# TinfoilHat0/Defending-Against-Backdoors-with-Robust-Learning-Rate

Measured on AMD Instinct MI355X. Metric: fl_rounds_per_sec, higher is better.
Workload: dtype fp32; 1 GPU; model=CNN_MNIST, dataset=fmnist (synthetic, 6000 samples/agent), num_agents=10, agents_per_gpu=10, num_corrupt=1, robustLR_threshold=4, aggr=avg, local_ep=2, global_batch=256, parallelism=dp1 (agent-sharded, RCCL all-gather)

## Files before the change

rlr_amd/ops/csrc/bindings.cpp:

```cpp
#include <torch/extension.h>
#include <c10/hip/HIPStream.h>

#include <algorithm>
#include <cstdint>
#include <vector>

#include "launchers.h"

#define CHK(x) TORCH_CHECK(x, #x)
#define CHK_CUDA(t)                                                      \
  TORCH_CHECK((t).is_cuda() &&                                           \
                  ((t).is_contiguous() ||                                \
                   (t).is_contiguous(torch::MemoryFormat::ChannelsLast)),\
              #t " must be cuda + dense")

static void* stream_of(const torch::Tensor& t) {
  return (void*)c10::hip::getCurrentHIPStream(t.device().index()).stream();
}

static bool layout_debug() {
  static int v = -1;
  if (v < 0) {
    const char* e = getenv("RLR_AMD_DEBUG_LAYOUT");
    v = (e && e[0] == '1') ? 1 : 0;
// ... 1326 lines not shown
                                  torch::Tensor dw_out,
                                  c10::optional<torch::Tensor> relu_y) {
  TORCH_CHECK(x.is_cuda());
  TORCH_CHECK(dw_out.is_contiguous() && dw_out.numel() == w.numel());
  return conv_bwd_core(x, w, dy, stride, pad, need_dx, dw_out, c10::nullopt,
                       relu_y);
}


std::tuple<torch::Tensor, torch::Tensor, torch::Tensor> batchnorm_fwd(
    torch::Tensor x, torch::Tensor w, torch::Tensor b,
    torch::Tensor running_mean, torch::Tensor running_var, double momentum,
    double eps, bool training, bool relu) {
  TORCH_CHECK(x.is_cuda());
  x = cl(x, "bn_fwd.x");
  int Nb = x.size(0), C = x.size(1), HW = x.size(2) * x.size(3);
  auto y = empty_cl({x.size(0), x.size(1), x.size(2), x.size(3)},
                    x.options());
  auto save_mean = torch::empty({C}, x.options().dtype(torch::kFloat));
  auto save_rstd = torch::empty({C}, x.options().dtype(torch::kFloat));
  auto scratch = torch::empty({(long)bn_scratch_floats(C)},
                              x.options().dtype(torch::kFloat));
  if (is_bf16(x))
    launch_bn_fwd_bf16(bfc(x), w.data_ptr<float>(), b.data_ptr<float>(),
                       running_mean.data_ptr<float>(),
                       running_var.data_ptr<float>(),
                       save_mean.data_ptr<float>(),
                       save_rstd.data_ptr<float>(), bfp(y),
                       scratch.data_ptr<float>(), Nb, C, HW,
                       (float)momentum, (float)eps, training ? 1 : 0,
                       relu ? 1 : 0, stream_of(x));
  else
    launch_bn_fwd(x.data_ptr<float>(), w.data_ptr<float>(),
                  b.data_ptr<float>(), running_mean.data_ptr<float>(),
                  running_var.data_ptr<float>(),
                  save_mean.data_ptr<float>(), save_rstd.data_ptr<float>(),
                  y.data_ptr<float>(), scratch.data_ptr<float>(), Nb, C,
                  HW, (float)momentum, (float)eps, training ? 1 : 0,
                  relu ? 1 : 0, stream_of(x));
  return {y, save_mean, save_rstd};
}

torch::Tensor batchnorm_bwd_into(torch::Tensor x, torch::Tensor w,
                                 torch::Tensor save_mean,
                                 torch::Tensor save_rstd, torch::Tensor dy,
                                 torch::Tensor dw_out, torch::Tensor db_out) {
  TORCH_CHECK(x.is_cuda());
  x = cl(x, "bn_bwd.x");
  dy = cl(dy, "bn_bwd.dy");
  int Nb = x.size(0), C = x.size(1), HW = x.size(2) * x.size(3);
  TORCH_CHECK(dw_out.is_contiguous() && dw_out.numel() == C);
  TORCH_CHECK(db_out.is_contiguous() && db_out.numel() == C);
  auto dx = empty_cl({x.size(0), x.size(1), x.size(2), x.size(3)},
                     x.options());
  auto scratch = torch::empty({(long)bn_scratch_floats(C)},
                              x.options().dtype(torch::kFloat));
  if (is_bf16(x))
    launch_bn_bwd_bf16(bfc(x), bfc(dy), w.data_ptr<float>(),
                       save_mean.data_ptr<float>(),
                       save_rstd.data_ptr<float>(),
                       scratch.data_ptr<float>(), bfp(dx),
                       dw_out.data_ptr<float>(), db_out.data_ptr<float>(),
                       Nb, C, HW, 1, stream_of(x));
  else
    launch_bn_bwd(x.data_ptr<float>(), dy.data_ptr<float>(),
                  w.data_ptr<float>(), save_mean.data_ptr<float>(),
                  save_rstd.data_ptr<float>(), scratch.data_ptr<float>(),
                  dx.data_ptr<float>(), dw_out.data_ptr<float>(),
                  db_out.data_ptr<float>(), Nb, C, HW, 1, stream_of(x));
  return dx;
}

std::tuple<torch::Tensor, torch::Tensor, torch::Tensor> batchnorm_bwd(
    torch::Tensor x, torch::Tensor w, torch::Tensor save_mean,
    torch::Tensor save_rstd, torch::Tensor dy) {
  auto f32 = x.options().dtype(torch::kFloat);
  auto dw = torch::empty({x.size(1)}, f32);
  auto db = torch::empty({x.size(1)}, f32);
  auto dx = batchnorm_bwd_into(x, w, save_mean, save_rstd, dy, dw, db);
  return {dx, dw, db};
}


void poison_set_u8(torch::Tensor data, torch::Tensor idxs,
                   torch::Tensor coords, int64_t value) {
  CHK_CUDA(data);
  int H = data.size(1), W = data.size(2);
  int C = data.dim() == 4 ? data.size(3) : 1;
  launch_poison_set_u8(data.data_ptr<uint8_t>(), idxs.data_ptr<int64_t>(),
                       idxs.numel(), coords.data_ptr<int>(),
                       coords.size(0), H, W, C, (int)value, stream_of(data));
}

void poison_set_f32(torch::Tensor data, torch::Tensor idxs,
                    torch::Tensor coords, double value) {
  CHK_CUDA(data);
  int H = data.size(2), W = data.size(3);
  launch_poison_set_f32(data.data_ptr<float>(), idxs.data_ptr<int64_t>(),
                        idxs.numel(), coords.data_ptr<int>(),
                        coords.size(0), H, W, (float)value, stream_of(data));
}

void poison_addwrap_u8(torch::Tensor data, torch::Tensor idxs,
                       torch::Tensor mask) {
  CHK_CUDA(data);
  launch_poison_addwrap_u8(data.data_ptr<uint8_t>(),
                           idxs.data_ptr<int64_t>(), idxs.numel(),
                           mask.data_ptr<uint8_t>(),
                           data.size(1) * data.size(2), stream_of(data));
}

void poison_subf(torch::Tensor data, torch::Tensor idxs,
                 torch::Tensor mask) {
  CHK_CUDA(data);
  long HW = data.numel() / data.size(0);
  launch_poison_subf(data.data_ptr<float>(), idxs.data_ptr<int64_t>(),
                     idxs.numel(), mask.data_ptr<uint8_t>(), (int)HW,
                     stream_of(data));
}

torch::Tensor normalize_u8(torch::Tensor raw, torch::Tensor mean,
                           torch::Tensor stdv) {
  TORCH_CHECK(raw.is_cuda() && raw.is_contiguous());
  long B = raw.size(0);
  int H = raw.size(1), W = raw.size(2);
  int C = raw.dim() == 4 ? raw.size(3) : 1;
  auto out = empty_cl({B, C, H, W}, raw.options().dtype(torch::kFloat32));
  launch_normalize_u8(raw.data_ptr<uint8_t>(), out.data_ptr<float>(), B, H,
                      W, C, mean.data_ptr<float>(), stdv.data_ptr<float>(),
                      stream_of(raw));
  return out;
}


std::vector<torch::Tensor> prep_conv_weights(
    std::vector<std::pair<torch::Tensor, int64_t>> items) {
  StepQueue q;
  std::vector<torch::Tensor> out;
  out.reserve(items.size());
  for (auto& it : items) out.push_back(q.wperm(it.first, it.second));
  q.flush();
  return out;
}

void feed_gather(torch::Tensor X, torch::Tensor Y, torch::Tensor sel,
                 torch::Tensor out_x, torch::Tensor out_y) {
  StepQueue q;
  q.gather_rows(X, sel, out_x);
  q.gather_rows(Y, sel, out_y);
  q.flush();
}

torch::Tensor conv_db(torch::Tensor dy) {
  TORCH_CHECK(dy.is_cuda() && dy.dim() == 4 && !is_bf16(dy));
  dy = cl(dy, "conv_db.dy");
  auto db = torch::empty({dy.size(1)}, dy.options());
  StepQueue(true).conv_db(dy, db);
  return db;
}

torch::Tensor splitk_reduce_dwperm(torch::Tensor ws, int64_t Kout, int64_t C,
                                   int64_t RS, int64_t SK) {
  CHK_CUDA(ws);
  TORCH_CHECK(ws.numel() >= conv_dwperm_ws_floats(Kout, C * RS, SK));
  auto dw = torch::empty({Kout * C * RS}, ws.options());
  StepQueue(true).splitk_reduce_dwperm(ws, dw, Kout, C, RS, SK, 0);
  return dw;
}

torch::Tensor splitk_reduce(torch::Tensor ws, int64_t M, int64_t N,
                            int64_t SK) {
  CHK_CUDA(ws);
  TORCH_CHECK(ws.numel() >= gemm_splitk_ws_floats(M, N, SK));
  auto C = torch::empty({M, N}, ws.options());
  if (!StepQueue(true).splitk_reduce(ws, C, c10::nullopt, M, N, N, SK, false))
    launch_splitk_reduce(ws.data_ptr<float>(), C.data_ptr<float>(), nullptr,
                         (int)M, (int)N, (int)N, (int)SK, 0, stream_of(ws));
  return C;
}

torch::Tensor conv_small_bwdw_reduce(torch::Tensor partials, int64_t Nb,
                                     int64_t C, int64_t Kout, int64_t R,
                                     int64_t S, int64_t OH, int64_t OW) {
  CHK_CUDA(partials);
  auto dw = torch::empty({Kout * C * R * S}, partials.options());
  StepQueue(true).conv_small_bwdw_reduce(partials, dw, Nb, C, Kout, R, S, OH,
                                         OW);
  return dw;
}

torch::Tensor colsum(torch::Tensor dy) {
  CHK_CUDA(dy);
  TORCH_CHECK(dy.dim() == 2);
  auto db = torch::empty({dy.size(1)}, dy.options());
  StepQueue(true).colsum(dy, db);
  return db;
}

torch::Tensor wperm(torch::Tensor w, int64_t kind) {
  TORCH_CHECK(w.is_cuda());
  return StepQueue(true).wperm(w, kind);
}

std::tuple<std::vector<int64_t>, int64_t> step_batch_plan_py(
    std::vector<int64_t> counts) {
  std::vector<int> c(counts.begin(), counts.end()), f(counts.size());
  int total = step_batch_plan(c.data(), (int)c.size(), f.data());
  return {std::vector<int64_t>(f.begin(), f.end()), (int64_t)total};
}

std::tuple<int64_t, int64_t> step_batch_lookup_py(std::vector<int64_t> counts,
                                                  int64_t block) {
  std::vector<int> c(counts.begin(), counts.end());
  int v = -1;
  int r = step_batch_lookup(c.data(), (int)c.size(), (int)block, &v);
  return {(int64_t)r, (int64_t)(r < 0 ? -1 : v)};
}

}

PYBIND11_MODULE(TORCH_EXTENSION_NAME, m) {
  m.def("relu_fwd", &relu_fwd);
  m.def("relu_bwd", &relu_bwd);
  m.def("add_relu_fwd", &add_relu_fwd);
  m.def("maxpool2x2_fwd", &maxpool2x2_fwd);
  m.def("maxpool2x2_bwd", &maxpool2x2_bwd);
  m.def("dropout_fwd", &dropout_fwd);
  m.def("dropout_fwd_dev", &dropout_fwd_dev);
  m.def("dropout_bwd", &dropout_bwd);
  m.def("gap_fwd", &gap_fwd);
  m.def("gap_bwd", &gap_bwd);
  m.def("cross_entropy_fwd", &cross_entropy_fwd);
  m.def("cross_entropy_bwd", &cross_entropy_bwd);
  m.def("eval_update", &eval_update);
  m.def("clipped_sgd_step", &clipped_sgd_step);
  m.def("pgd_project", &pgd_project);
  m.def("delta64", &delta64);
  m.def("gather_grads", &gather_grads);
  m.def("fused_avg_rlr_apply", &fused_avg_rlr_apply, py::arg("U"),
        py::arg("w"), py::arg("params"), py::arg("rlr"), py::arg("thresh"),
        py::arg("slr"), py::arg("noise_std"), py::arg("seed"),
        py::arg("offset"), py::arg("want_lr"), py::arg("divisor") = 0.0);
  m.def("rlr_vote", &rlr_vote);
  m.def("agg_avg", &agg_avg, py::arg("U"), py::arg("w"),
        py::arg("divisor") = 0.0);
  m.def("agg_sign", &agg_sign);
  m.def("agg_comed", &agg_comed);
  m.def("apply_update", &apply_update);
  m.def("agg_orderstat", &agg_orderstat);
  m.def("orderstat_rlr_apply", &orderstat_rlr_apply);
  m.def("orderstat_max_k", &orderstat_max_k);
  m.def("bulyan_trim", &bulyan_trim);
  m.def("bulyan_rlr_apply", &bulyan_rlr_apply);
  m.def("bulyan_max_k", &bulyan_max_k);
  m.def("pairwise_sqdist", &pairwise_sqdist);
  m.def("pairdist_max_k", &pairdist_max_k);
  m.def("pairdist_chunks", &pairdist_chunks);
  m.def("pairdist_ws_doubles", &pairdist_ws_doubles);
  m.def("rows_add_", &rows_add_);
  m.def("gram_rows", &gram_rows);
  m.def("foolsgold_weights", &foolsgold_weights);
  m.def("foolsgold_max_k", &foolsgold_max_k);
  m.def("geomed_sqdist", &geomed_sqdist);
  m.def("geomed_weights", &geomed_weights);
  m.def("geomed_max_k", &geomed_max_k);
  m.def("geomed_chunks", &geomed_chunks);
  m.def("geomed_ws_doubles", &geomed_ws_doubles);
  m.def("rownorm_partials", &rownorm_partials);
  m.def("row_norms", &row_norms, py::arg("U"), py::arg("ws") = py::none());
  m.def("rowclip_", &rowclip_, py::arg("U"), py::arg("value"),
        py::arg("median_mode"), py::arg("ws") = py::none());
  m.def("rownorm_chunks", &rownorm_chunks);
  m.def("rownorm_ws_doubles", &rownorm_ws_doubles);
  m.def("gemm", &gemm);
  m.def("gemm_bf16", &gemm_bf16);
  m.def("nhwc_flatten", &nhwc_flatten);
  m.def("nhwc_unflatten", &nhwc_unflatten);
  m.def("linear_fwd", &linear_fwd);
  m.def("linear_bwd", &linear_bwd);
  m.def("conv2d_fwd", &conv2d_fwd, py::arg("x"), py::arg("w"), py::arg("b"),
        py::arg("stride"), py::arg("pad"), py::arg("relu"),
        py::arg("wt") = py::none());
  m.def("conv2d_pool_fwd", &conv2d_pool_fwd, py::arg("x"), py::arg("w"),
        py::arg("b"), py::arg("stride"), py::arg("pad"),
        py::arg("wt") = py::none());
  m.def("conv_pool_fused_ok", &conv_pool_fused_ok);
  m.def("conv_fwd_res_plan", [](int C, int H, int W, int OH, int OW, int R) {
    ConvFwdResPlan p = conv_fwd_res_plan(C, H, W, OH, OW, R);
    return std::make_tuple(p.tile_rows, p.tiles, p.mi, p.lds_rows,
                           p.lds_bytes);
  });
  m.def("conv2d_bwd", &conv2d_bwd);
  m.def("conv2d_bwd_into", &conv2d_bwd_into, py::arg("x"), py::arg("w"),
        py::arg("dy"), py::arg("stride"), py::arg("pad"), py::arg("need_dx"),
        py::arg("dw_out"), py::arg("db_out"), py::arg("relu_y"),
        py::arg("wp") = py::none(), py::arg("queue") = py::none());
  m.def("linear_bwd_into", &linear_bwd_into, py::arg("x"), py::arg("w"),
        py::arg("dy"), py::arg("dw_out"), py::arg("db_out"),
        py::arg("need_dx"), py::arg("queue") = py::none());
  m.def("dropout_relu_bwd", &dropout_relu_bwd);
  m.def("batchnorm_bwd_into", &batchnorm_bwd_into);
  m.def("conv2d_bwd_wdx_into", &conv2d_bwd_wdx_into);
  m.def("gemm_f32_splitk", &gemm_f32_splitk);
  m.def("conv_bwd_weight_splitk", &conv_bwd_weight_splitk);
  m.def("conv_bwd_weight_bf16_splitk", &conv_bwd_weight_bf16_splitk);
  m.def("conv_db_chunks", &conv_db_chunks);
  m.def("gemm_splitk_ws_floats", &gemm_splitk_ws_floats);
  m.def("conv_bwd_weight_ws_floats", &conv_bwd_weight_ws_floats);
  m.def("conv_dwperm_ws_floats", &conv_dwperm_ws_floats);
  m.def("conv_db_ws_floats", &conv_db_ws_floats);
  m.def("flat_norm_scratch_floats", &flat_norm_scratch_floats);
  m.def("conv_bwdw_tap_ws_slabs", [](int64_t Nb, int64_t C, int64_t Kout) {
    int S, G, chunks;
    int slabs = conv_bwdw_tap_ws_slabs((int)Nb, (int)C, (int)Kout, &S, &G,
                                       &chunks);
    return std::make_tuple(S, G, chunks, slabs);
  });
  m.def("conv_tap_fwd_ok", [](int a, int b, int c, int d, int e, int f,
                              int g, int h) {
    return conv_tap_fwd_ok(a, b, c, d, e, f, g, h) != 0;
  });
  m.def("conv_tap_fwd_w4_ok", [](int a, int b, int c, int d, int e, int f,
                                 int g, int h) {
    return conv_tap_fwd_w4_ok(a, b, c, d, e, f, g, h) != 0;
  });
  m.def("conv_tap_bwdd_s2_ok", [](int a, int b, int c, int d, int e, int f,
                                  int g, int h) {
    return conv_tap_bwdd_s2_ok(a, b, c, d, e, f, g, h) != 0;
  });
  m.def("conv_bwdw_tap_ok", [](int a, int b, int c, int d, int e, int f,
                               int g, int h) {
    return conv_bwdw_tap_ok(a, b, c, d, e, f, g, h) != 0;
  });
  m.def("conv_bwdw_tap_s2_ok", [](int a, int b, int c, int d, int e, int f,
                                  int g, int h) {
    return conv_bwdw_tap_s2_ok(a, b, c, d, e, f, g, h) != 0;
  });
  m.def("pool_flatten_dropout_fwd", &pool_flatten_dropout_fwd);
  m.def("flatten_dropout_fwd", &flatten_dropout_fwd);
  m.def("dropout_unflatten_pool_bwd_relu", &dropout_unflatten_pool_bwd_relu);
  m.def("fc_head_step", &fc_head_step, py::arg("h1"), py::arg("w"),
        py::arg("b"), py::arg("labels"), py::arg("dloss"), py::arg("p"),
        py::arg("state"), py::arg("site"), py::arg("dw_out"),
        py::arg("db_out"), py::arg("queue") = py::none());
  py::class_<StepQueue>(m, "StepQueue")
      .def(py::init<>())
      .def("flush", &StepQueue::flush)
      .def("pending", &StepQueue::pending)
      .def("conv_db", &StepQueue::conv_db)
      .def("splitk_reduce_dwperm", &StepQueue::splitk_reduce_dwperm,
           py::arg("ws"), py::arg("dw"), py::arg("Kout"), py::arg("C"),
           py::arg("RS"), py::arg("SK"), py::arg("ws_offset") = 0)
      .def("splitk_reduce", &StepQueue::splitk_reduce)
      .def("colsum", &StepQueue::colsum)
      .def("conv_small_bwdw_reduce", &StepQueue::conv_small_bwdw_reduce)
      .def("wperm", &StepQueue::wperm)
      .def("gather_rows", &StepQueue::gather_rows)
      .def("add_u64", &StepQueue::add_u64);
  m.def("prep_conv_weights", &prep_conv_weights);
  m.def("feed_gather", &feed_gather);
  m.def("conv_db", &conv_db);
  m.def("splitk_reduce_dwperm", &splitk_reduce_dwperm);
  m.def("splitk_reduce", &splitk_reduce);
  m.def("conv_small_bwdw_reduce", &conv_small_bwdw_reduce);
  m.def("colsum", &colsum);
  m.def("wperm", &wperm);
  m.def("step_batch_max_roles", &step_batch_max_roles);
  m.def("step_batch_plan", &step_batch_plan_py);
  m.def("step_batch_lookup", &step_batch_lookup_py);
  m.def("pool_seam_fused_ok", &pool_seam_fused_ok);
  m.def("fc_head_fused_ok", &fc_head_fused_ok);
  m.def("fc_head_ws_floats", &fc_head_ws_floats);
  m.def("add_", &add_inplace);
  m.def("add_relu_bwd_", &add_relu_bwd_);
  m.def("gap_bwd_relu", &gap_bwd_relu);
  m.def("maxpool2x2_bwd_relu", &maxpool2x2_bwd_relu);
  m.def("batchnorm_fwd", &batchnorm_fwd);
  m.def("batchnorm_bwd", &batchnorm_bwd);
  m.def("poison_set_u8", &poison_set_u8);
  m.def("poison_set_f32", &poison_set_f32);
  m.def("poison_addwrap_u8", &poison_addwrap_u8);
  m.def("poison_subf", &poison_subf);
  m.def("normalize_u8", &normalize_u8);
}
```

rlr_amd/ops/csrc/gemm_f32.hip:

```cpp
#include "common.h"
#include "launchers.h"
#include "tail_math.h"

typedef float f32x4 __attribute__((ext_vector_type(4)));

constexpr int BM = 128, BN = 64, BK = 32;
constexpr int LDA_S = BK + 2;
constexpr int LDB_S = BN + 16;

template <bool VEC, bool AT = false, bool BT = false>
__global__ __launch_bounds__(256)
void gemm_f32_k(const float* __restrict__ A, const float* __restrict__ B,
                float* __restrict__ C, const float* __restrict__ bias,
                int M, int N, int K, int lda, int ldb, int ldc,
                long k_per_chunk, int relu, int direct_out) {
  __shared__ float A_lds[2][BM * LDA_S];
  __shared__ float B_lds[2][BK * LDB_S];

  const int m_blk = blockIdx.x * BM;
  const int n_blk = blockIdx.y * BN;
  const long k_lo = (long)blockIdx.z * k_per_chunk;
  const long k_hi = min((long)K, k_lo + k_per_chunk);

  const int t = threadIdx.x;
  const int wave = t >> 6, lane = t & 63;
  const int wr = wave >> 1, wc = wave & 1;
  const int l15 = lane & 15, l4 = lane >> 4;

  f32x4 acc[4][2];
#pragma unroll
  for (int mi = 0; mi < 4; ++mi)
#pragma unroll
    for (int ni = 0; ni < 2; ++ni) acc[mi][ni] = {0.f, 0.f, 0.f, 0.f};

  const int am = t >> 3;
  const int ak = (t & 7) * 4;
  const int bk = t >> 4;
  const int bn = (t & 15) * 4;

  float4 ra[4], rb[2];
  const int tak = t >> 3;
  const int tam = (t & 7) * 4;
  const int tbn = t >> 3;
  const int tbk = (t & 7) * 4;
  auto stage_load = [&](long k0) {
    if (AT) {
#pragma unroll
      for (int j = 0; j < 4; ++j) {
        long gk = k0 + tak;
        long gm = m_blk + tam + j * 32;
        float v0 = 0.f, v1 = 0.f, v2 = 0.f, v3 = 0.f;
        if (gk < k_hi) {
          long base = gk * (long)lda + gm;
          if (VEC && gm + 3 < M) {
            const float4 q = *(const float4*)(A + base);
            v0 = q.x; v1 = q.y; v2 = q.z; v3 = q.w;
          } else {
            if (gm + 0 < M) v0 = A[base + 0];
            if (gm + 1 < M) v1 = A[base + 1];
            if (gm + 2 < M) v2 = A[base + 2];
            if (gm + 3 < M) v3 = A[base + 3];
          }
        }
        ra[j] = {v0, v1, v2, v3};
      }
    } else {
#pragma unroll
      for (int j = 0; j < 4; ++j) {
        int m = am + j * 32;
        long gm = m_blk + m;
        float v0 = 0.f, v1 = 0.f, v2 = 0.f, v3 = 0.f;
        if (gm < M) {
          long base = gm * (long)lda + k0 + ak;
          if (VEC && k0 + ak + 3 < k_hi) {
            const float4 q = *(const float4*)(A + base);
            v0 = q.x; v1 = q.y; v2 = q.z; v3 = q.w;
          } else {
            if (k0 + ak + 0 < k_hi) v0 = A[base + 0];
            if (k0 + ak + 1 < k_hi) v1 = A[base + 1];
            if (k0 + ak + 2 < k_hi) v2 = A[base + 2];
            if (k0 + ak + 3 < k_hi) v3 = A[base + 3];
          }
        }
        ra[j] = {v0, v1, v2, v3};
      }
    }
    if (BT) {
#pragma unroll
      for (int j = 0; j < 2; ++j) {
        long gn = n_blk + tbn + j * 32;
        long gk = k0 + tbk;
        float v0 = 0.f, v1 = 0.f, v2 = 0.f, v3 = 0.f;
        if (gn < N) {
          long base = gn * (long)ldb + gk;
          if (VEC && gk + 3 < k_hi) {
            const float4 q = *(const float4*)(B + base);
            v0 = q.x; v1 = q.y; v2 = q.z; v3 = q.w;
          } else {
            if (gk + 0 < k_hi) v0 = B[base + 0];
            if (gk + 1 < k_hi) v1 = B[base + 1];
            if (gk + 2 < k_hi) v2 = B[base + 2];
            if (gk + 3 < k_hi) v3 = B[base + 3];
          }
        }
        rb[j] = {v0, v1, v2, v3};
      }
    } else {
#pragma unroll
      for (int j = 0; j < 2; ++j) {
        long gk = k0 + bk + j * 16;
        float v0 = 0.f, v1 = 0.f, v2 = 0.f, v3 = 0.f;
        if (gk < k_hi) {
          long base = gk * (long)ldb + n_blk + bn;
          if (VEC && n_blk + bn + 3 < N) {
            const float4 q = *(const float4*)(B + base);
            v0 = q.x; v1 = q.y; v2 = q.z; v3 = q.w;
          } else {
            if (n_blk + bn + 0 < N) v0 = B[base + 0];
            if (n_blk + bn + 1 < N) v1 = B[base + 1];
            if (n_blk + bn + 2 < N) v2 = B[base + 2];
            if (n_blk + bn + 3 < N) v3 = B[base + 3];
          }
        }
        rb[j] = {v0, v1, v2, v3};
      }
    }
  };
  auto stage_write = [&](int buf) {
    if (AT) {
#pragma unroll
      for (int j = 0; j < 4; ++j) {
        const float v[4] = {ra[j].x, ra[j].y, ra[j].z, ra[j].w};
#pragma unroll
        for (int e = 0; e < 4; ++e)
          A_lds[buf][(tam + j * 32 + e) * LDA_S + tak] = v[e];
      }
    } else {
#pragma unroll
      for (int j = 0; j < 4; ++j) {
        float* dst = &A_lds[buf][(am + j * 32) * LDA_S + ak];
        ((float2*)dst)[0] = {ra[j].x, ra[j].y};
        ((float2*)dst)[1] = {ra[j].z, ra[j].w};
      }
    }
    if (BT) {
#pragma unroll
      for (int j = 0; j < 2; ++j) {
        const float v[4] = {rb[j].x, rb[j].y, rb[j].z, rb[j].w};
#pragma unroll
        for (int e = 0; e < 4; ++e)
          B_lds[buf][(tbk + e) * LDB_S + tbn + j * 32] = v[e];
      }
    } else {
#pragma unroll
      for (int j = 0; j < 2; ++j)
        *(float4*)&B_lds[buf][(bk + j * 16) * LDB_S + bn] = rb[j];
    }
  };

  stage_load(k_lo);
  stage_write(0);
  if (k_lo + BK < k_hi) stage_load(k_lo + BK);
  __syncthreads();

  int buf = 0;
  for (long k0 = k_lo; k0 < k_hi; k0 += BK) {
    if (k0 + BK < k_hi) {
      stage_write(buf ^ 1);
      if (k0 + 2 * BK < k_hi) stage_load(k0 + 2 * BK);
    }
    const float* Abuf = A_lds[buf];
    const float* Bbuf = B_lds[buf];
#pragma unroll
    for (int kk = 0; kk < BK / 4; ++kk) {
      float a_frag[4], b_frag[2];
#pragma unroll
      for (int mi = 0; mi < 4; ++mi)
        a_frag[mi] = Abuf[(wr * 64 + mi * 16 + l15) * LDA_S + kk * 4 + l4];
#pragma unroll
      for (int ni = 0; ni < 2; ++ni)
        b_frag[ni] = Bbuf[(kk * 4 + l4) * LDB_S + wc * 32 + ni * 16 + l15];
#pragma unroll
      for (int mi = 0; mi < 4; ++mi)
#pragma unroll
        for (int ni = 0; ni < 2; ++ni)
          acc[mi][ni] = __builtin_amdgcn_mfma_f32_16x16x4f32(
              a_frag[mi], b_frag[ni], acc[mi][ni], 0, 0, 0);
    }
    __syncthreads();
    buf ^= 1;
  }

#pragma unroll
  for (int mi = 0; mi < 4; ++mi) {
#pragma unroll
    for (int ni = 0; ni < 2; ++ni) {
      int col = n_blk + wc * 32 + ni * 16 + l15;
      if (col >= N) continue;
#pragma unroll
      for (int r = 0; r < 4; ++r) {
        int row = m_blk + wr * 64 + mi * 16 + l4 * 4 + r;
        if (row >= M) continue;
        float v = acc[mi][ni][r];
        if (direct_out) {
          if (bias) v += bias[col];
          if (relu) v = fmaxf(v, 0.f);
          C[(long)row * ldc + col] = v;
        } else {
          C[((long)blockIdx.z * M + row) * N + col] = v;
        }
      }
    }
  }
}

__global__ void splitk_reduce_wave_k(const float* __restrict__ ws,
                                     float* __restrict__ C,
                                     const float* __restrict__ bias, int M,
                                     int N, int ldc, int SK, int relu) {
  long n_out = (long)M * N;
  long i = blockIdx.x * (long)(blockDim.x / kWave) + threadIdx.x / kWave;
  int lane = threadIdx.x % kWave;
  if (i >= n_out) return;
  float acc = 0.f;
  for (int z = lane; z < SK; z += kWave) acc += ws[(long)z * n_out + i];
#pragma unroll
  for (int off = 32; off > 0; off >>= 1) acc += __shfl_down(acc, off, kWave);
  if (lane == 0) {
    int col = i % N;
    if (bias) acc += bias[col];
    if (relu) acc = fmaxf(acc, 0.f);
    C[(i / N) * (long)ldc + col] = acc;
  }
}


__global__ void gemm_small_k(const float* __restrict__ A,
                             const float* __restrict__ B,
                             float* __restrict__ C,
                             const float* __restrict__ bias, int M, int N,
                             int K, int lda, int ldb, int ldc, int relu,
                             int layout) {
  long n_out = (long)M * N;
  long stride = (long)gridDim.x * blockDim.x;
  for (long i = (long)blockIdx.x * blockDim.x + threadIdx.x; i < n_out;
       i += stride) {
    int n = (int)(i % N);
    int m = (int)(i / N);
    const float* a = layout == 1 ? A + m : A + (long)m * lda;
    const long astep = layout == 1 ? lda : 1;
    const float* b = layout == 2 ? B + (long)n * ldb : B + n;
    const long bstep = layout == 2 ? 1 : ldb;
    float acc = dot_rot4(K, [&](int k) { return a[k * astep]; },
                         [&](int k) { return b[k * bstep]; });
    if (bias) acc += bias[n];
    if (relu) acc = fmaxf(acc, 0.f);
    C[(long)m * ldc + n] = acc;
  }
}

__global__ void gemm_small_wave_k(const float* __restrict__ A,
                                  const float* __restrict__ B,
                                  float* __restrict__ C,
                                  const float* __restrict__ bias, int M,
                                  int N, int K, int lda, int ldb, int ldc,
                                  int relu, int layout) {
  long out = blockIdx.x * (long)(blockDim.x / kWave) + threadIdx.x / kWave;
  int lane = threadIdx.x % kWave;
  if (out >= (long)M * N) return;
  int n = (int)(out % N);
  int m = (int)(out / N);
  const float* a = layout == 1 ? A + m : A + (long)m * lda;
  const long astep = layout == 1 ? lda : 1;
  const float* b = layout == 2 ? B + (long)n * ldb : B + n;
  const long bstep = layout == 2 ? 1 : ldb;
  float acc = dot_wave_partial(K, lane, [&](int k) { return a[k * astep]; },
                               [&](int k) { return b[k * bstep]; });
  acc = wave_tree_down(acc);
  if (lane == 0) {
    if (bias) acc += bias[n];
    if (relu) acc = fmaxf(acc, 0.f);
    C[(long)m * ldc + n] = acc;
  }
}

extern "C" {

int gemm_f32_splitk(int M, int N, int K) {
  static long target = -1;
  if (target < 0) {
    const char* e = getenv("RLR_GEMM_SK_TARGET");
    target = e ? atol(e) : 256;
  }
  long tiles = ((M + BM - 1) / BM) * (long)((N + BN - 1) / BN);
  if (tiles >= 192 || K <= 2 * BK) return 1;
  long want = (target + tiles - 1) / tiles;
  long max_chunks = (K + BK - 1) / BK;
  long sk = want < max_chunks ? want : max_chunks;
  return (int)(sk < 1 ? 1 : (sk > 192 ? 192 : sk));
}

long gemm_splitk_ws_floats(int M, int N, int SK) {
  if (SK == 1) return 0;
  return (long)(SK + splitk_stage1_slabs(SK)) * M * N;
}

int launch_gemm_f32_main(const float* A, const float* B, float* C,
                         const float* bias, float* ws, int M, int N, int K,
                         int lda, int ldb, int ldc, int SK, int relu,
                         int layout, void* s) {
  hipStream_t st = (hipStream_t)s;
  if ((long)M * N * K <= 8'000'000 && (long)M * N <= 65536) {
    if (K >= 32) {
      int wpb = kBlock / kWave;
      gemm_small_wave_k<<<((long)M * N + wpb - 1) / wpb, kBlock, 0, st>>>(
          A, B, C, bias, M, N, K, lda, ldb, ldc, relu, layout);
    } else {
      gemm_small_k<<<grid_for((long)M * N), kBlock, 0, st>>>(
          A, B, C, bias, M, N, K, lda, ldb, ldc, relu, layout);
    }
    return 0;
  }
  dim3 grid((M + BM - 1) / BM, (N + BN - 1) / BN, SK);
  long k_per_chunk = SK == 1 ? (long)K
                             : ((((long)K + SK - 1) / SK + BK - 1) / BK) * BK;
  bool vec = (lda % 4 == 0) && (ldb % 4 == 0);
  float* out = SK == 1 ? C : ws;
  if (layout == 1) {
    if (vec)
      gemm_f32_k<true, true, false><<<grid, 256, 0, st>>>(
          A, B, out, bias, M, N, K, lda, ldb, ldc, k_per_chunk, relu,
          SK == 1);
    else
      gemm_f32_k<false, true, false><<<grid, 256, 0, st>>>(
          A, B, out, bias, M, N, K, lda, ldb, ldc, k_per_chunk, relu,
          SK == 1);
  } else if (layout == 2) {
    if (vec)
      gemm_f32_k<true, false, true><<<grid, 256, 0, st>>>(
          A, B, out, bias, M, N, K, lda, ldb, ldc, k_per_chunk, relu,
          SK == 1);
    else
      gemm_f32_k<false, false, true><<<grid, 256, 0, st>>>(
          A, B, out, bias, M, N, K, lda, ldb, ldc, k_per_chunk, relu,
          SK == 1);
  } else if (vec)
    gemm_f32_k<true><<<grid, 256, 0, st>>>(A, B, out, bias, M, N, K, lda,
                                           ldb, ldc, k_per_chunk, relu,
                                           SK == 1);
  else
    gemm_f32_k<false><<<grid, 256, 0, st>>>(A, B, out, bias, M, N, K, lda,
                                            ldb, ldc, k_per_chunk, relu,
                                            SK == 1);
  return SK > 1;
}

StepRole splitk_partial_role(const float* ws, float* out, long n_out, int S,
                             int zstride) {
  int chunks = (S + zstride - 1) / zstride;
  StepRole r{};
  r.kind = kRoleSplitkPartial;
  r.gx = grid_for(n_out * chunks);
  r.gy = 1;
  r.count = r.gx;
  r.splitk_partial.ws = ws;
  r.splitk_partial.out = out;
  r.splitk_partial.n_out = n_out;
  r.splitk_partial.S = S;
  r.splitk_partial.zstride = zstride;
  return r;
}

static StepRole splitk_reduce_role(const float* ws, float* C,
                                   const float* bias, int M, int N, int ldc,
                                   int SK, int relu) {
  StepRole r{};
  r.kind = kRoleSplitkReduce;
  r.gx = grid_for((long)M * N);
  r.gy = 1;
  r.count = r.gx;
  r.splitk_reduce.ws = ws;
  r.splitk_reduce.C = C;
  r.splitk_reduce.bias = bias;
  r.splitk_reduce.M = M;
  r.splitk_reduce.N = N;
  r.splitk_reduce.ldc = ldc;
  r.splitk_reduce.SK = SK;
  r.splitk_reduce.relu = relu;
  return r;
}

int splitk_reduce_roles(const float* ws, float* C, const float* bias, int M,
                        int N, int ldc, int SK, int relu, StepRole* l1,
                        StepRole* l2) {
  long n_out = (long)M * N;
  if (SK > kSplitKFold && n_out <= 262144) {
    int chunks = splitk_stage1_slabs(SK);
    float* ws2 = const_cast<float*>(ws) + (long)SK * n_out;
    *l1 = splitk_partial_role(ws, ws2, n_out, SK, kSplitKFold);
    *l2 = splitk_reduce_role(ws2, C, bias, M, N, ldc, chunks, relu);
    return 2;
  }
  if (n_out <= 8192 && SK >= 16) return 0;
  *l1 = splitk_reduce_role(ws, C, bias, M, N, ldc, SK, relu);
  return 1;
}

StepRole colsum_role(const float* dY, float* db, int M, int N) {
  int wpb = kBlock / kWave;
  StepRole r{};
  r.kind = kRoleColsum;
  r.gx = (N + wpb - 1) / wpb;
  r.gy = 1;
  r.count = r.gx;
  r.colsum.dY = dY;
  r.colsum.db = db;
  r.colsum.M = M;
  r.colsum.N = N;
  return r;
}

void launch_splitk_reduce(const float* ws, float* C, const float* bias,
                          int M, int N, int ldc, int SK, int relu, void* s) {
  StepRole a, b;
  int levels = splitk_reduce_roles(ws, C, bias, M, N, ldc, SK, relu, &a, &b);
  if (levels == 0) {
    long n_out = (long)M * N;
    int wpb = kBlock / kWave;
    splitk_reduce_wave_k<<<(n_out + wpb - 1) / wpb, kBlock, 0,
                           (hipStream_t)s>>>(ws, C, bias, M, N, ldc, SK,
                                             relu);
    return;
  }
  launch_step_role(&a, s);
  if (levels == 2) launch_step_role(&b, s);
}
}
```

rlr_amd/ops/csrc/launchers.h:

```cpp
#pragma once
#include <cstdint>

struct ConvDbStage1Args {
  const float* dy; float* partials; long M; int Kout, chunks, K_blk;
};
struct ConvDbStage2Args { const float* partials; float* db; int Kout, chunks; };
struct SplitkPartialArgs {
  const float* ws; float* out; long n_out; int S, zstride;
};
struct SplitkReduceArgs {
  const float* ws; float* C; const float* bias; int M, N, ldc, SK, relu;
};
struct SplitkReduceDwpermArgs {
  const float* ws; float* dw; int Kout, C, RS, SK;
};
struct ConvSmallBwdwReduceArgs {
  const float* partials; float* dw; int KO, C, RS, chunks;
};
struct ColsumArgs { const float* dY; float* db; int M, N; };
struct FcHeadReduceArgs {
  const float *gl, *d2, *row_loss; float *dw, *db, *loss;
  int B, H, C, dw_blocks, db_blocks, dw_wave;
};
struct WpermArgs { const float* w; float* out; int Kout, C, RS; };
struct GatherRowsArgs {
  const uint32_t* src; const long* sel; uint32_t* dst; long rows;
  int row_words, vec, src_rows;
};
struct AddU64Args { unsigned long long* p; unsigned long long delta; };
enum StepRoleKind {
  kRoleConvDbStage1 = 0,
  kRoleConvDbStage2,
  kRoleSplitkPartial,
  kRoleSplitkReduce,
  kRoleSplitkReduceDwperm,
  kRoleConvSmallBwdwReduce,
  kRoleColsum,
  kRoleFcHeadReduce,
  kRoleWpermRscKo,
  kRoleWpermRskoC,
  kRoleGatherRows,
  kRoleAddU64,
  kStepRoleKinds,
};
struct StepRole {
  int kind;
  int first;
  int count;
  int gx, gy;
  union {
    ConvDbStage1Args conv_db_stage1;
    ConvDbStage2Args conv_db_stage2;
    SplitkPartialArgs splitk_partial;
    SplitkReduceArgs splitk_reduce;
    SplitkReduceDwpermArgs splitk_reduce_dwperm;
    ConvSmallBwdwReduceArgs conv_small_bwdw_reduce;
    ColsumArgs colsum;
    FcHeadReduceArgs fc_head_reduce;
    WpermArgs wperm;
    GatherRowsArgs gather_rows;
    AddU64Args add_u64;
  };
};
static_assert(sizeof(StepRole) <= 104, "16 of them are kernel arguments");
constexpr int kStepMaxRoles = 16;

struct ConvFwdResPlan {
  int tile_rows, tiles, mi, lds_rows;
  long lds_bytes;
};

extern "C" {
int launch_step_role(const StepRole* r, void* s);
int step_batch_max_roles();
int step_batch_plan(const int* counts, int n, int* first);
int step_batch_lookup(const int* counts, int n, int block, int* vblock);
int launch_step_batch(const StepRole* roles, int n, void* s);
StepRole step_role_gather_rows(const void* src, const long* sel, void* dst,
                               long rows, int row_words, int src_rows);
StepRole step_role_add_u64(unsigned long long* p, unsigned long long delta);
void launch_relu_fwd(const float* x, float* y, long n, void* s);
void launch_relu_bwd(const float* y, const float* dy, float* dx, long n,
                     void* s);
void launch_add_relu(const float* a, const float* b, float* y, long n,
                     void* s);
void launch_add_relu_bwd(float* a, const float* b, const float* y, long n,
                         void* s);
void launch_add_relu_bwd_bf16(unsigned short* a, const unsigned short* b,
                              const unsigned short* y, long n, void* s);
void launch_add_inplace(float* a, const float* b, long n, void* s);
void launch_add_inplace_bf16(unsigned short* a, const unsigned short* b,
                             long n, void* s);
void launch_maxpool2x2_fwd(const float* x, float* y, uint8_t* idx, long B,
                           int H, int W, int OH, int OW, int C, void* s);
void launch_maxpool2x2_bwd(const float* dy, const uint8_t* idx, float* dx,
                           long B, int H, int W, int OH, int OW, int C,
                           void* s);
void launch_maxpool2x2_bwd_relu(const float* dy, const uint8_t* idx,
                                const float* relu_pooled, float* dx, long B,
                                int H, int W, int OH, int OW, int C,
                                void* s);
void launch_maxpool2x2_fwd_bf16(const unsigned short* x, unsigned short* y,
                                uint8_t* idx, long B, int H, int W, int OH,
                                int OW, int C, void* s);
void launch_maxpool2x2_bwd_bf16(const unsigned short* dy,
                                const uint8_t* idx, unsigned short* dx,
                                long B, int H, int W, int OH, int OW, int C,
                                void* s);
void launch_gap_fwd(const float* x, float* y, long B, int HW, int C,
                    void* s);
void launch_gap_bwd(const float* dy, float* dx, long B, int HW, int C,
                    void* s);
void launch_gap_bwd_relu(const float* dy, const float* y, float* dx, long B,
                         int HW, int C, void* s);
void launch_dropout_fwd(const float* x, float* y, uint8_t* mask, long n,
                        float p, uint64_t seed, uint64_t offset, void* s);
void launch_dropout_fwd_dev(const float* x, float* y, uint8_t* mask, long n,
                            float p, const unsigned long long* state,
                            int site, void* s);
void launch_dropout_bwd(const float* dy, const uint8_t* mask, float* dx,
                        long n, float p, void* s);
void launch_dropout_relu_bwd(const float* dy, const uint8_t* mask,
                             const float* y, float* dx, long n, float p,
                             void* s);
void launch_ce_fwd(const float* logits, const long* labels, float* softmax,
                   float* row_loss, float* loss_out, int B, int C, void* s);
void launch_ce_bwd(const float* softmax, const long* labels,
                   const float* dloss, float* dlogits, int B, int C,
                   void* s);
void launch_eval_update(const float* logits, const long* labels, float* conf,
                        double* loss_sum, int B, int C, int num_classes,
                        void* s);
void launch_nhwc_flatten(const float* in, float* out, long B, int C, int H,
                         int W, void* s);
void launch_nhwc_unflatten(const float* in, float* out, long B, int C,
                           int H, int W, void* s);
void launch_relu_fwd_bf16(const unsigned short* x, unsigned short* y,
                          long n, void* s);
void launch_relu_bwd_bf16(const unsigned short* y, const unsigned short* dy,
                          unsigned short* dx, long n, void* s);
void launch_add_relu_bf16(const unsigned short* a, const unsigned short* b,
                          unsigned short* y, long n, void* s);
void launch_dropout_fwd_dev_bf16(const unsigned short* x, unsigned short* y,
                                 uint8_t* mask, long n, float p,
                                 const unsigned long long* state, int site,
                                 void* s);
void launch_dropout_bwd_bf16(const unsigned short* dy, const uint8_t* mask,
                             unsigned short* dx, long n, float p, void* s);
void launch_gap_fwd_bf16(const unsigned short* x, unsigned short* y, long B,
                         int HW, int C, void* s);
void launch_gap_bwd_bf16(const unsigned short* dy, unsigned short* dx,
                         long B, int HW, int C, void* s);
void launch_gap_bwd_relu_bf16(const unsigned short* dy,
                              const unsigned short* y, unsigned short* dx,
                              long B, int HW, int C, void* s);
void launch_nhwc_flatten_bf16(const unsigned short* in, unsigned short* out,
                              long B, int C, int H, int W, void* s);
void launch_nhwc_unflatten_bf16(const unsigned short* in,
                                unsigned short* out, long B, int C, int H,
                                int W, void* s);
int pool_seam_fused_ok(int C, int H, int W);
void launch_pool_flatten_dropout_fwd(const float* x, float* pooled,
                                     uint8_t* idx, float* d, uint8_t* mask,
                                     long B, int H, int W, int C, float p,
                                     const unsigned long long* state,
                                     int site, void* s);
void launch_flatten_dropout_fwd(const float* pooled, float* d, uint8_t* mask,
                                long B, int OH, int OW, int C, float p,
                                const unsigned long long* state, int site,
                                void* s);
void launch_dropout_unflatten_pool_bwd_relu(const float* g,
                                            const uint8_t* mask,
                                            const uint8_t* idx,
                                            const float* pooled, float* dx,
                                            long B, int H, int W, int C,
                                            float p, void* s);
int fc_head_fused_ok(int B, int H, int C);
long fc_head_ws_floats(int B, int H, int C);
void launch_fc_head_rows(const float* h1, const float* w, const float* bias,
                         const long* labels, const float* dloss, float* ws,
                         float* g_h1, int B, int H, int C, float p,
                         const unsigned long long* state, int site,
                         void* s);
StepRole fc_head_reduce_role(const float* ws, float* dw, float* db,
                             float* loss, int B, int H, int C);
long flat_norm_scratch_floats();
void launch_clipped_sgd(float* p, const float* g, float* v, float* scratch,
                        float lr, float mu, float max_norm, long n, void* s);
void launch_pgd_project(float* p, const float* t0, float* scratch, float clip,
                        long n, void* s);
void launch_delta64(const float* p, const double* t0, double* out, long n,
                    void* s);
void launch_gather_grads(const float* const* srcs, const long* offs,
                         const long* lens, int count, float* flat, void* s);
void launch_fused_avg_rlr_apply(const double* U, const double* w, int K,
                                long n, double inv_wsum, int mode_rlr,
                                double thresh, double slr, float* params,
                                double* lr_out, double noise_std,
                                uint64_t seed, uint64_t offset, void* s);
void launch_rlr_vote(const double* U, int K, long n, double thresh,
                     double slr, double* lr, void* s);
void launch_agg_avg(const double* U, const double* w, int K, long n,
                    double inv_wsum, double* out, void* s);
void launch_agg_sign(const double* U, int K, long n, double* out, void* s);
void launch_agg_comed(const double* U, int K, long n, double* out, void* s);
void launch_apply_update(float* params, const double* agg, const double* lr,
                         double slr, long n, void* s);
int orderstat_max_k();
void launch_agg_orderstat(const double* U, int K, long n, int lo, int hi,
                          double inv_cnt, double* out, double* lr_out,
                          double thresh, double slr, void* s);
void launch_orderstat_rlr_apply(const double* U, int K, long n, int lo,
                                int hi, double inv_cnt, int mode_rlr,
                                double thresh, double slr, float* params,
                                double* lr_out, void* s);
int bulyan_max_k();
void launch_bulyan_trim(const double* U, const int* perm, int K, int theta,
                        int beta, long n, double* out, double* lr_out,
                        double thresh, double slr, void* s);
void launch_bulyan_rlr_apply(const double* U, const int* perm, int K,
                             int theta, int beta, long n, int mode_rlr,
                             double thresh, double slr, float* params,
                             double* lr_out, void* s);
int pairdist_max_k();
int pairdist_chunks(int K, long n);
long pairdist_ws_doubles(int K, long n);
void launch_pairwise_sqdist(const double* U, int K, long n, double* ws,
                            double* D, void* s);
void launch_gram_rows(const double* H, const long* rows, int K, long n,
                      double* ws, double* G, void* s);
int foolsgold_max_k();
void launch_rows_add(double* H, const long* rows, const double* U, int K,
                     long n, void* s);
void launch_foolsgold_weights(const double* G, int K, double kappa,
                              double* cs, double* alpha, void* s);
int geomed_max_k();
int geomed_chunks(int K, long n);
long geomed_ws_doubles(int K, long n);
void launch_geomed_sqdist(const double* U, const double* a, int K, long n,
                          double* ws, double* d2, void* s);
void launch_geomed_weights(const double* U, int K, long n, int iters,
                           double nu, double* ws, double* a, double* d2,
                           void* s);
int rownorm_chunks(int K, long n);
long rownorm_ws_doubles(int K, long n);
void launch_rownorm_partials(const double* U, int K, long n, double* ws,
                             void* s);
void launch_row_norms(const double* U, int K, long n, double* ws,
                      double* norm, void* s);
void launch_rowclip(double* U, int K, long n, double value, int median_mode,
                    double* ws, double* norm, double* scale, double* tau,
                    void* s);
int gemm_f32_splitk(int M, int N, int K);
long gemm_splitk_ws_floats(int M, int N, int SK);
int launch_gemm_f32_main(const float* A, const float* B, float* C,
                         const float* bias, float* ws, int M, int N, int K,
                         int lda, int ldb, int ldc, int SK, int relu,
                         int layout, void* s);
int splitk_reduce_roles(const float* ws, float* C, const float* bias, int M,
                        int N, int ldc, int SK, int relu, StepRole* l1,
                        StepRole* l2);
void launch_splitk_reduce(const float* ws, float* C, const float* bias,
                          int M, int N, int ldc, int SK, int relu, void* s);
StepRole splitk_partial_role(const float* ws, float* out, long n_out, int S,
                             int zstride);
StepRole colsum_role(const float* dY, float* db, int M, int N);
void launch_gemm_bf16(const unsigned short* A, const unsigned short* B,
                      float* C, const float* bias, unsigned short* C16,
                      float* ws, int M, int N, int K, int lda, int ldb,
                      int ldc, int SK, int relu, void* s);
void launch_conv_fwd(const float* x, const float* wt, const float* bias,
                     float* y, int Nb, int C, int H, int W, int Kout, int R,
                     int S, int OH, int OW, int stride, int pad, int relu,
                     void* s);
ConvFwdResPlan conv_fwd_res_plan(int C, int H, int W, int OH, int OW, int R);
int conv_pool_fused_ok(int C, int H, int W, int Kout, int R, int S,
                       int stride, int pad);
void launch_conv_pool_fwd(const float* x, const float* wt, const float* bias,
                          float* pooled, uint8_t* idx, int Nb, int C, int H,
                          int W, int Kout, int R, int S, void* s);
void launch_conv_bwd_data_relu(const float* dy, const float* wp,
                               float* dx, const float* relu_y, int Nb,
                               int C, int H, int W, int Kout, int R, int S,
                               int OH, int OW, int stride, int pad,
                               void* s);
int conv_bwd_weight_splitk(int Kout, int Ncrs, long Kdim);
long conv_bwd_weight_ws_floats(int Kout, int Ncrs, int SK);
int conv_small_bwdw_chunks(long Kdim);
void launch_conv_bwd_weight(const float* dy, const float* x, float* dw,
                            float* ws, int SK, int Nb, int C, int H, int W,
                            int Kout, int R, int S, int OH, int OW,
                            int stride, int pad, void* s);
void launch_conv_bwd_weight_main(const float* dy, const float* x, float* ws,
                                 int SK, int Nb, int C, int H, int W,
                                 int Kout, int R, int S, int OH, int OW,
                                 int stride, int pad, void* s);
int conv_bwd_weight_combine_roles(float* ws, float* dw, int SK, int Nb,
                                  int C, int Kout, int R, int S, int OH,
                                  int OW, StepRole* l1, StepRole* l2);
int splitk_reduce_dwperm_roles(const float* ws, float* dw, int Kout, int C,
                               int RS, int SK, StepRole* l1, StepRole* l2);
void conv_db_roles(const float* dy, float* db, float* partials, int Nb,
                   int Kout, int OHW, StepRole* l1, StepRole* l2);
StepRole wperm_role(int kind, const float* w, float* out, int Kout, int C,
                    int RS);
int conv_db_chunks(long M, int Kout);
long conv_db_ws_floats(int Kout);
long conv_dwperm_ws_floats(int Kout, int Ncrs, int SK);
int conv_bwd_weight_bf16_splitk(int Kout, int Ncrs, long Kdim);
void launch_conv_fwd_bf16(const unsigned short* x, const unsigned short* wt,
                          const float* bias, unsigned short* y, int Nb,
                          int C, int H, int W, int Kout, int R, int S,
                          int OH, int OW, int stride, int pad, int relu,
                          void* s);
void launch_conv_bwd_data_bf16_relu(const unsigned short* dy,
                                    const unsigned short* wp,
                                    unsigned short* dx,
                                    const unsigned short* relu_y, int Nb,
                                    int C, int H, int W, int Kout, int R,
                                    int S, int OH, int OW, int stride,
                                    int pad, void* s);
void launch_conv_bwd_weight_bf16(const unsigned short* dy,
                                 const unsigned short* x, float* dw,
                                 float* ws, int SK, int Nb, int C, int H,
                                 int W, int Kout, int R, int S, int OH,
                                 int OW, int stride, int pad, void* s);
void launch_wperm_rsc_ko_bf16(const float* w, unsigned short* out, int Kout,
                              int C, int RS, void* s);
void launch_wperm_rsko_c_bf16(const float* w, unsigned short* out, int Kout,
                              int C, int RS, void* s);
void launch_conv_db_bf16(const unsigned short* dy, float* db,
                         float* partials, int Nb, int Kout, int OHW,
                         void* s);
int conv_bwdw_tap_ok(int C, int H, int W, int Kout, int R, int S,
                     int stride, int pad);
int conv_bwdw_tap_s2_ok(int C, int H, int W, int Kout, int R, int S,
                        int stride, int pad);
int conv_bwdw_tap_ws_slabs(int Nb, int C, int Kout, int* S_out, int* G_out,
                           int* chunks_out);
void launch_conv_bwdw_tap_bf16(const unsigned short* dy,
                               const unsigned short* x, float* dw,
                               float* ws, int Nb, int C, int H, int W,
                               int Kout, void* st);
void launch_conv_bwdw_tap_s2_bf16(const unsigned short* dy,
                                  const unsigned short* x, float* dw,
                                  float* ws, int Nb, int C, int H, int W,
                                  int Kout, void* st);
int conv_tap_fwd_ok(int Cin, int H, int W, int Cout, int R, int S,
                    int stride, int pad);
void launch_conv_tap_fwd_bf16(const unsigned short* x,
                              const unsigned short* wt, const float* bias,
                              unsigned short* y,
                              const unsigned short* relu_y, int Nb,
                              int Cin, int H, int W, int Cout, int relu,
                              int flip, void* st);
int conv_tap_fwd_w4_ok(int Cin, int H, int W, int Cout, int R, int S,
                       int stride, int pad);
void launch_conv_tap_fwd_w4_bf16(const unsigned short* x,
                                 const unsigned short* wt,
                                 const float* bias, unsigned short* y,
                                 const unsigned short* relu_y, int Nb,
                                 int Cin, int Cout, int relu, int flip,
                                 void* st);
int conv_tap_bwdd_s2_ok(int C, int H, int W, int KO, int R, int S,
                        int stride, int pad);
void launch_conv_tap_bwdd_s2_bf16(const unsigned short* dy,
                                  const unsigned short* wp,
                                  unsigned short* dx,
                                  const unsigned short* relu_y, int Nb,
                                  int KO, int H, int W, int C, void* st);
int bn_scratch_floats(int C);
void launch_bn_fwd(const float* x, const float* w, const float* b,
                   float* running_mean, float* running_var, float* save_mean,
                   float* save_rstd, float* y, float* scratch, int Nb,
                   int C, int HW, float momentum, float eps, int training,
                   int relu, void* s);
void launch_bn_fwd_bf16(const unsigned short* x, const float* w,
                        const float* b, float* running_mean,
                        float* running_var, float* save_mean,
                        float* save_rstd, unsigned short* y, float* scratch,
                        int Nb, int C, int HW, float momentum, float eps,
                        int training, int relu, void* s);
void launch_bn_bwd(const float* x, const float* dy, const float* w,
                   const float* save_mean, const float* save_rstd,
                   float* scratch, float* dx, float* dw, float* db, int Nb,
                   int C, int HW, int training, void* s);
void launch_bn_bwd_bf16(const unsigned short* x, const unsigned short* dy,
                        const float* w, const float* save_mean,
                        const float* save_rstd, float* scratch,
                        unsigned short* dx, float* dw, float* db, int Nb,
                        int C, int HW, int training, void* s);
void launch_poison_set_u8(uint8_t* data, const long* idxs, int B,
                          const int* coords, int P, int H, int W, int C,
                          int value, void* s);
void launch_poison_set_f32(float* data, const long* idxs, int B,
                           const int* coords, int P, int H, int W,
                           float value, void* s);
void launch_poison_addwrap_u8(uint8_t* data, const long* idxs, int B,
                              const uint8_t* mask, int HW, void* s);
void launch_poison_subf(float* data, const long* idxs, int B,
                        const uint8_t* mask, int HW, void* s);
void launch_normalize_u8(const uint8_t* raw, float* out, long B, int H,
                         int W, int C, const float* mean, const float* stdv,
                         void* s);
void launch_conv_bwd_weight_bf16_ex(const unsigned short* dy,
                                    const unsigned short* x, float* dw,
                                    float* ws, int SK, int variant, int Nb,
                                    int C, int H, int W, int Kout, int R,
                                    int S, int OH, int OW, int stride,
                                    int pad, void* s);
}
```

Measured before the change: 6.233 rounds/s.

## Add short-K fp32 GEMM kernel that preloads all K tiles into registers

Adds a specialized MFMA GEMM kernel for cases where each split-K chunk spans 3 to 5 BK tiles. All global loads for the chunk are issued up front into registers, then staged into double-buffered LDS as compute proceeds, so load latency is not serialized per tile. It is dispatched automatically from the main fp32 GEMM launcher, with an env var to disable it. The cost is higher register pressure from holding all tile fragments, which may lower occupancy.

```diff
diff --git a/rlr_amd/ops/csrc/bindings.cpp b/rlr_amd/ops/csrc/bindings.cpp
--- a/rlr_amd/ops/csrc/bindings.cpp
+++ b/rlr_amd/ops/csrc/bindings.cpp
@@ -1652,6 +1652,7 @@
   m.def("batchnorm_bwd_into", &batchnorm_bwd_into);
   m.def("conv2d_bwd_wdx_into", &conv2d_bwd_wdx_into);
   m.def("gemm_f32_splitk", &gemm_f32_splitk);
+  m.def("gemm_f32_shortk_tiles", &gemm_f32_shortk_tiles);
   m.def("conv_bwd_weight_splitk", &conv_bwd_weight_splitk);
   m.def("conv_bwd_weight_bf16_splitk", &conv_bwd_weight_bf16_splitk);
   m.def("conv_db_chunks", &conv_db_chunks);
diff --git a/rlr_amd/ops/csrc/gemm_f32.hip b/rlr_amd/ops/csrc/gemm_f32.hip
--- a/rlr_amd/ops/csrc/gemm_f32.hip
+++ b/rlr_amd/ops/csrc/gemm_f32.hip
@@ -209,6 +209,197 @@
         } else {
           C[((long)blockIdx.z * M + row) * N + col] = v;
         }
+      }
+    }
+  }
+}
+
+constexpr int kShortKMaxTiles = 5;
+
+__device__ __forceinline__ float4 sk_load(const float* __restrict__ P,
+                                          long row, long ld, long v0,
+                                          bool row_ok, long lim) {
+  const bool full = row_ok && v0 + 3 < lim;
+  float4 q = *(const float4*)(P + (full ? row * ld + v0 : 0));
+  if (row_ok && !full && v0 < lim) {
+    const float* r = P + row * ld + v0;
+    q.x = r[0];
+    q.y = v0 + 1 < lim ? r[1] : 0.f;
+    q.z = v0 + 2 < lim ? r[2] : 0.f;
+    q.w = 0.f;
+  }
+  return q;
+}
+
+__device__ __forceinline__ float4 sk_mask(float4 q, bool row_ok, long v0,
+                                          long lim) {
+  const bool keep = row_ok && v0 < lim;
+  return {keep ? q.x : 0.f, keep ? q.y : 0.f, keep ? q.z : 0.f,
+          keep ? q.w : 0.f};
+}
+
+template <int NT, bool AT, bool BT>
+__device__ __forceinline__ void shortk_chunk(
+    const float* __restrict__ A, const float* __restrict__ B, int M, int N,
+    int lda, int ldb, int m_blk, int n_blk, long k_lo, long k_hi,
+    float (&A_lds)[2][BM * LDA_S], float (&B_lds)[2][BK * LDB_S],
+    f32x4 (&acc)[4][2]) {
+  const int t = threadIdx.x;
+  const int wave = t >> 6, lane = t & 63;
+  const int wr = wave >> 1, wc = wave & 1;
+  const int l15 = lane & 15, l4 = lane >> 4;
+  const int a_r = t >> 3, a_v = (t & 7) * 4;
+  const int b_r = BT ? t >> 3 : t >> 4;
+  const int b_v = BT ? (t & 7) * 4 : (t & 15) * 4;
+
+  float4 ra[NT][4], rb[NT][2];
+#pragma unroll
+  for (int i = 0; i < NT; ++i) {
+    const long k0 = k_lo + i * BK;
+#pragma unroll
+    for (int j = 0; j < 4; ++j) {
+      if (AT)
+        ra[i][j] = sk_load(A, k0 + a_r, lda, m_blk + a_v + j * 32,
+                           k0 + a_r < k_hi, M);
+      else
+        ra[i][j] = sk_load(A, m_blk + a_r + j * 32, lda, k0 + a_v,
+                           m_blk + a_r + j * 32 < M, k_hi);
+    }
+#pragma unroll
+    for (int j = 0; j < 2; ++j) {
+      if (BT)
+        rb[i][j] = sk_load(B, n_blk + b_r + j * 32, ldb, k0 + b_v,
+                           n_blk + b_r + j * 32 < N, k_hi);
+      else
+        rb[i][j] = sk_load(B, k0 + b_r + j * 16, ldb, n_blk + b_v,
+                           k0 + b_r + j * 16 < k_hi, N);
+    }
+  }
+
+#pragma unroll
+  for (int i = 0; i <= NT; ++i) {
+#pragma unroll
+    for (int half = 0; half < 2; ++half) {
+      if (i > 0) {
+        const float* Abuf = A_lds[(i - 1) & 1];
+        const float* Bbuf = B_lds[(i - 1) & 1];
+#pragma unroll
+        for (int kk = half * (BK / 8); kk < (half + 1) * (BK / 8); ++kk) {
+          float a_frag[4], b_frag[2];
+#pragma unroll
+          for (int mi = 0; mi < 4; ++mi)
+            a_frag[mi] =
+                Abuf[(wr * 64 + mi * 16 + l15) * LDA_S + kk * 4 + l4];
+#pragma unroll
+          for (int ni = 0; ni < 2; ++ni)
+            b_frag[ni] =
+                Bbuf[(kk * 4 + l4) * LDB_S + wc * 32 + ni * 16 + l15];
+#pragma unroll
+          for (int mi = 0; mi < 4; ++mi)
+#pragma unroll
+            for (int ni = 0; ni < 2; ++ni)
+              acc[mi][ni] = __builtin_amdgcn_mfma_f32_16x16x4f32(
+                  a_frag[mi], b_frag[ni], acc[mi][ni], 0, 0, 0);
+        }
+      }
+      if (half == 0 && i < NT) {
+        const long k0 = k_lo + i * BK;
+        float* Aw = A_lds[i & 1];
+        float* Bw = B_lds[i & 1];
+#pragma unroll
+        for (int j = 0; j < 4; ++j) {
+          if (AT) {
+            const float4 q = sk_mask(ra[i][j], k0 + a_r < k_hi,
+                                     m_blk + a_v + j * 32, M);
+            const float v[4] = {q.x, q.y, q.z, q.w};
+#pragma unroll
+            for (int e = 0; e < 4; ++e)
+              Aw[(a_v + j * 32 + e) * LDA_S + a_r] = v[e];
+          } else {
+            const float4 q = sk_mask(ra[i][j], m_blk + a_r + j * 32 < M,
+                                     k0 + a_v, k_hi);
+            float* dst = &Aw[(a_r + j * 32) * LDA_S + a_v];
+            ((float2*)dst)[0] = {q.x, q.y};
+            ((float2*)dst)[1] = {q.z, q.w};
+          }
+        }
+#pragma unroll
+        for (int j = 0; j < 2; ++j) {
+          if (BT) {
+            const float4 q = sk_mask(rb[i][j], n_blk + b_r + j * 32 < N,
+                                     k0 + b_v, k_hi);
+            const float v[4] = {q.x, q.y, q.z, q.w};
+#pragma unroll
+            for (int e = 0; e < 4; ++e)
+              Bw[(b_v + e) * LDB_S + b_r + j * 32] = v[e];
+          } else {
+            const float4 q = sk_mask(rb[i][j], k0 + b_r + j * 16 < k_hi,
+                                     n_blk + b_v, N);
+            *(float4*)&Bw[(b_r + j * 16) * LDB_S + b_v] = q;
+          }
+        }
+      }
+    }
+    if (i < NT) __syncthreads();
+  }
+}
+
+template <int NT, bool AT, bool BT, typename... Args>
+__device__ __forceinline__ void shortk_dispatch(int nt, Args&&... args) {
+  if (nt == NT) {
+    shortk_chunk<NT, AT, BT>(args...);
+  } else if constexpr (NT > 1) {
+    shortk_dispatch<NT - 1, AT, BT>(nt, args...);
+  }
+}
+
+template <int T, bool AT, bool BT>
+__global__ __launch_bounds__(256)
+void gemm_f32_shortk_k(const float* __restrict__ A,
+                       const float* __restrict__ B, float* __restrict__ C,
+                       const float* __restrict__ bias, int M, int N, int K,
+                       int lda, int ldb, int ldc, long k_per_chunk, int relu,
+                       int direct_out) {
+  __shared__ float A_lds[2][BM * LDA_S];
+  __shared__ float B_lds[2][BK * LDB_S];
+
+  const int m_blk = blockIdx.x * BM;
+  const int n_blk = blockIdx.y * BN;
+  const long k_lo = (long)blockIdx.z * k_per_chunk;
+  const long k_hi = min((long)K, k_lo + k_per_chunk);
+  const int nt = k_hi > k_lo ? (int)((k_hi - k_lo + BK - 1) / BK) : 0;
+
+  f32x4 acc[4][2];
+#pragma unroll
+  for (int mi = 0; mi < 4; ++mi)
+#pragma unroll
+    for (int ni = 0; ni < 2; ++ni) acc[mi][ni] = {0.f, 0.f, 0.f, 0.f};
+
+  shortk_dispatch<T, AT, BT>(nt, A, B, M, N, lda, ldb, m_blk, n_blk, k_lo,
+                             k_hi, A_lds, B_lds, acc);
+
+  const int t = threadIdx.x;
+  const int lane = t & 63, wave = t >> 6;
+  const int wr = wave >> 1, wc = wave & 1;
+  const int l15 = lane & 15, l4 = lane >> 4;
+  const int ldo = direct_out ? ldc : N;
+  float* __restrict__ O = direct_out ? C : C + (long)blockIdx.z * M * N;
+#pragma unroll
+  for (int mi = 0; mi < 4; ++mi) {
+#pragma unroll
+    for (int ni = 0; ni < 2; ++ni) {
+      int col = n_blk + wc * 32 + ni * 16 + l15;
+      if (col >= N) continue;
+#pragma unroll
+      for (int r = 0; r < 4; ++r) {
+        int row = m_blk + wr * 64 + mi * 16 + l4 * 4 + r;
+        if (row >= M) continue;
+        float v = acc[mi][ni][r];
+        if (direct_out) {
+          if (bias) v += bias[col];
+          if (relu) v = fmaxf(v, 0.f);
+        }
+        O[(long)row * ldo + col] = v;
       }
     }
   }
@@ -305,12 +496,45 @@
   return (long)(SK + splitk_stage1_slabs(SK)) * M * N;
 }
 
+static bool gemm_f32_tiny(int M, int N, int K) {
+  return (long)M * N * K <= 8'000'000 && (long)M * N <= 65536;
+}
+
+int gemm_f32_shortk_tiles(int M, int N, int K, int SK, int lda, int ldb) {
+  if (gemm_f32_tiny(M, N, K)) return 0;
+  if (lda % 4 != 0 || ldb % 4 != 0) return 0;
+  long k_per_chunk = SK == 1 ? (long)K
+                             : ((((long)K + SK - 1) / SK + BK - 1) / BK) * BK;
+  if (k_per_chunk <= 2 * BK || k_per_chunk > kShortKMaxTiles * BK) return 0;
+  return (int)((k_per_chunk + BK - 1) / BK);
+}
+
+static void launch_gemm_f32_shortk(const float* A, const float* B, float* out,
+                                   const float* bias, int M, int N, int K,
+                                   int lda, int ldb, int ldc, dim3 grid,
+                                   long k_per_chunk, int relu, int direct_out,
+                                   int layout, hipStream_t st) {
+  constexpr int T = kShortKMaxTiles;
+  if (layout == 1)
+    gemm_f32_shortk_k<T, true, false><<<grid, 256, 0, st>>>(
+        A, B, out, bias, M, N, K, lda, ldb, ldc, k_per_chunk, relu,
+        direct_out);
+  else if (layout == 2)
+    gemm_f32_shortk_k<T, false, true><<<grid, 256, 0, st>>>(
+        A, B, out, bias, M, N, K, lda, ldb, ldc, k_per_chunk, relu,
+        direct_out);
+  else
+    gemm_f32_shortk_k<T, false, false><<<grid, 256, 0, st>>>(
+        A, B, out, bias, M, N, K, lda, ldb, ldc, k_per_chunk, relu,
+        direct_out);
+}
+
 int launch_gemm_f32_main(const float* A, const float* B, float* C,
                          const float* bias, float* ws, int M, int N, int K,
                          int lda, int ldb, int ldc, int SK, int relu,
                          int layout, void* s) {
   hipStream_t st = (hipStream_t)s;
-  if ((long)M * N * K <= 8'000'000 && (long)M * N <= 65536) {
+  if (gemm_f32_tiny(M, N, K)) {
     if (K >= 32) {
       int wpb = kBlock / kWave;
       gemm_small_wave_k<<<((long)M * N + wpb - 1) / wpb, kBlock, 0, st>>>(
@@ -326,6 +550,13 @@
                              : ((((long)K + SK - 1) / SK + BK - 1) / BK) * BK;
   bool vec = (lda % 4 == 0) && (ldb % 4 == 0);
   float* out = SK == 1 ? C : ws;
+  const char* no_shortk = getenv("RLR_AMD_NO_GEMM_SHORTK");
+  if (!(no_shortk && no_shortk[0] == '1') &&
+      gemm_f32_shortk_tiles(M, N, K, SK, lda, ldb)) {
+    launch_gemm_f32_shortk(A, B, out, bias, M, N, K, lda, ldb, ldc, grid,
+                           k_per_chunk, relu, SK == 1, layout, st);
+    return SK > 1;
+  }
   if (layout == 1) {
     if (vec)
       gemm_f32_k<true, true, false><<<grid, 256, 0, st>>>(
diff --git a/rlr_amd/ops/csrc/launchers.h b/rlr_amd/ops/csrc/launchers.h
--- a/rlr_amd/ops/csrc/launchers.h
+++ b/rlr_amd/ops/csrc/launchers.h
@@ -253,6 +253,7 @@
                     void* s);
 int gemm_f32_splitk(int M, int N, int K);
 long gemm_splitk_ws_floats(int M, int N, int SK);
+int gemm_f32_shortk_tiles(int M, int N, int K, int SK, int lda, int ldb);
 int launch_gemm_f32_main(const float* A, const float* B, float* C,
                          const float* bias, float* ws, int M, int N, int K,
                          int lda, int ldb, int ldc, int SK, int relu,
```

Measured after the change: 6.344 rounds/s (median of 6 runs). +1.8%, better.
